# JoeMWatson/input-inference-for-control

Hardware: AMD Instinct MI355X
Metric: i2c timestep-messages/sec (cell-iterations/s = B*T*EM-iters/s), pendulum T=200 B=4096 per GPU (higher is better)
Workload: dtype f64; 1 GPU; pendulum_known_quad cubature i2c (nx=2, nu=1, nz=4), T=200, B=4096 trajectories per GPU, global batch 4096, CubatureQuadrature(1,0,0), alpha0=100, tol=0; batch_per_gpu=4096, horizon=200, parallelism=batch-sharded x1, no collective in the EM loop, kernels=one lane per trajectory

## Files before the change

### input-inference-for-control_amd/csrc/i2c_cell.hpp

```cpp
#pragma once
#include <stdint.h>
#include <type_traits>
#include "../../include/i2c_hip.h"
#include "i2c_linalg.hpp"
#include "i2c_models.hpp"
#include "i2c_random.hpp"

namespace i2c {

template <typename R> struct Rule {
  R sf;
  R w0;
  R wi;
  R W;
  int unit;
  int gh_degree, gh_points;
  R gh_x[I2C_MAX_GH_DEGREE], gh_w[I2C_MAX_GH_DEGREE];
};

template <class M> struct PerTraj : M {};
template <class M> struct is_per_traj : std::false_type {};
template <class M> struct is_per_traj<PerTraj<M>> : std::true_type {};
template <typename R, bool PER_TRAJ> struct ParamsB {};
template <typename R> struct ParamsB<R, true> {
// ... 142 lines not shown
  I2C_HD static constexpr int dep(int k) { return M::obs_dep(k); }
};
template <class M> struct TermStruct {
  I2C_HD static constexpr int lin(int k) { return M::term_lin(k); }
  I2C_HD static constexpr int dep(int k) { return M::term_dep(k); }
};
template <class M> struct MeasStruct {
  I2C_HD static constexpr int lin(int k) { return M::meas_lin(k); }
  I2C_HD static constexpr int dep(int k) { return M::meas_dep(k); }
};
template <int DIN> struct DenseStruct {
  I2C_HD static constexpr int lin(int) { return -1; }
  I2C_HD static constexpr int dep(int) { return DIN - 1; }
};

template <class M, class ST, int DIN, int DOUT, bool CROSS, bool UNITW = false, bool HANDOFF = false, typename R, class F>
I2C_FN void sp_transform(const Rule<R>& rule, const R* m, const R* Sin, const R* L, const F& f, R* my, R* Sy,
                         R* Sxy, const PolyTab<R>* tab = nullptr) {
  static_assert(!HANDOFF || (CROSS && ST::lin(0) < 0 && ST::dep(0) == DIN - 1 && ST::lin(DOUT - 1) < 0 && ST::dep(DOUT - 1) == DIN - 1),
                "the hand-off of the differences is the dense callback's");
  constexpr int NA = M::NA, NA1 = NA > 0 ? NA : 1;
  R s0[NA1], c0[NA1];
#pragma unroll
  for (int a = 0; a < NA; ++a) {
    if (tab)
      r_sincos(m[M::ang(a)], *tab, &s0[a], &c0[a]);
    else
      r_sincos(m[M::ang(a)], &s0[a], &c0[a]);
  }
  R y0[DOUT];
  f(m, s0, c0, y0);
  constexpr bool NOISE = carries_noise<F>::value;
  static_assert(!NOISE || (!HANDOFF && ST::lin(0) < 0 && ST::dep(0) == DIN - 1), "a noise term rides on a dense callback, whose every column is evaluated");
  R q0[NOISE ? sym(DOUT) : 1], qs[NOISE ? sym(DOUT) : 1];
  if constexpr (NOISE) {
    f.noise(m, s0, c0, q0);
#pragma unroll
    for (int i = 0; i < sym(DOUT); ++i) qs[i] = R(0);
  }
  R A[DOUT];
#pragma unroll
  for (int k = 0; k < DOUT; ++k) A[k] = R(0);
#pragma unroll
// ... 17 lines not shown
          xm[i] = m[i];
        } else {
          const R d = rule.sf * L[tri(i, j)];
          xp[i] = m[i] + d;
          xm[i] = m[i] - d;
        }
      }
      R sp[NA1], cp[NA1], sm[NA1], cm[NA1];
#pragma unroll
      for (int q = 0; q < NA; ++q) {
        if (M::ang(q) < j) {
          sp[q] = sm[q] = s0[q];
          cp[q] = cm[q] = c0[q];
        } else {
          R sd, cd;
          if (tab)
            r_sincos(rule.sf * L[tri(M::ang(q), j)], *tab, &sd, &cd);
          else
            r_sincos_small(rule.sf * L[tri(M::ang(q), j)], &sd, &cd);
          sp[q] = s0[q] * cd + c0[q] * sd;
          cp[q] = c0[q] * cd - s0[q] * sd;
          sm[q] = s0[q] * cd - c0[q] * sd;
          cm[q] = c0[q] * cd + s0[q] * sd;
        }
      }
      R yp[DOUT], ym[DOUT];
      f(xp, sp, cp, yp);
      f(xm, sm, cm, ym);
      if constexpr (NOISE) {
        R qp[sym(DOUT)], qm[sym(DOUT)];
        f.noise(xp, sp, cp, qp);
        f.noise(xm, sm, cm, qm);
#pragma unroll
        for (int i = 0; i < sym(DOUT); ++i) qs[i] += qp[i] + qm[i];
      }
#pragma unroll
      for (int k = 0; k < DOUT; ++k) {
        a[k] = (yp[k] - y0[k]) + (ym[k] - y0[k]);
// ... 70 lines not shown
    R v = mu[i];
#pragma unroll
    for (int k = 0; k < DZ; ++k) v += Sxz[i * DZ + k] * q[k];
    mu[i] = v;
    sched_fence<(DZ >= 8)>();
  }
#pragma unroll
  for (int i = 0; i < DX; ++i)
#pragma unroll
    for (int j = 0; j <= i; ++j) {
      R v = S[tri(i, j)];
#pragma unroll
      for (int k = 0; k < DZ; ++k) v -= Sxz[i * DZ + k] * Sxz[j * DZ + k];
      S[tri(i, j)] = v;
    }
  return ok;
}

template <int N, typename R> I2C_FN R pdf_ratio(R* S, const R* delta, bool* ok, const PolyTab<R>* tab = nullptr) {
  R rinv[N], q[N];
  *ok = chol<N>(S, rinv);
#pragma unroll
  for (int i = 0; i < N; ++i) q[i] = delta[i];
  fsub<N>(S, rinv, q);
  R maha = R(0);
#pragma unroll
  for (int i = 0; i < N; ++i) maha += q[i] * q[i];
  (void)tab;
  return r_exp(R(-0.5) * maha);
}
// ... 248 lines not shown
  return (int)__builtin_amdgcn_mbcnt_hi(~0u, __builtin_amdgcn_mbcnt_lo(~0u, 0u));
#endif
}
template <int GRID> I2C_FN bool grid_writer() {
  if constexpr (GRID == GRID_WAVE) return grid_lane() == 0;
  else return true;
}
template <int GRID> I2C_FN void grid_read_before_write() {
#ifdef I2C_HOST_SIM
  if constexpr (GRID == GRID_WAVE) grid_sim_sync();
#endif
}
template <class M, int DIN, int DOUT, bool CROSS, typename R, class F>
I2C_FN void grid_transform_wave(const Rule<R>& rule, const R* m, const R* L, const F& f, R* my, R* Sy, R* Sxy);

template <int GRID, class M, class ST, int DIN, int DOUT, bool CROSS, bool UNITW = false, bool HANDOFF = false, typename R, class F>
I2C_FN void transform(const Rule<R>& rule, const R* m, const R* Sin, const R* L, const F& f, R* my, R* Sy, R* Sxy,
                      const PolyTab<R>* tab = nullptr) {
  static_assert(!HANDOFF || GRID == 0, "the hand-off of the differences is the sigma-point rule's (sp_transform)");
  if constexpr (GRID == GRID_WAVE) {
    grid_transform_wave<M, DIN, DOUT, CROSS>(rule, m, L, f, my, Sy, Sxy);
  } else if constexpr (GRID != 0) {
    if constexpr (DIN <= 3) {
      if (rule.gh_degree == 3) return grid_transform_ct<M, 3, DIN, DOUT, CROSS>(rule, m, L, f, my, Sy, Sxy);
      if (rule.gh_degree == 4) return grid_transform_ct<M, 4, DIN, DOUT, CROSS>(rule, m, L, f, my, Sy, Sxy);
      if (rule.gh_degree == 2) return grid_transform_ct<M, 2, DIN, DOUT, CROSS>(rule, m, L, f, my, Sy, Sxy);
    }
    grid_transform<M, DIN, DOUT, CROSS>(rule, m, L, f, my, Sy, Sxy);
  } else
    sp_transform<M, ST, DIN, DOUT, CROSS, UNITW, HANDOFF>(rule, m, Sin, L, f, my, Sy, Sxy, tab);
}


template <typename R, typename S = R> struct FwdArgs {
  const S* prior;
  S* fwd;
  S* prior_out;
  const R* x0;
  const R* sig_x0;
  const R* z;
  const R* alpha;
  const R* alpha_cell;
  const uint8_t* ff;
  int32_t* status;
  const uint8_t* expert;
};

struct NoRelease {
  static constexpr bool ON = false, GAIN = false;
  int chunk_len;
  I2C_HD inline void release() const {}
  I2C_HD inline void release_if(int, int) const {}
};
struct ChunkRelease {
  static constexpr bool ON = true, GAIN = false;
  int chunk_len;
  I2C_HD inline void release() const {
#if defined(__HIP_DEVICE_COMPILE__)
    __builtin_amdgcn_fence(__ATOMIC_RELEASE, "workgroup");
    __builtin_amdgcn_s_waitcnt(0x0F70);
    __builtin_amdgcn_s_barrier();
#endif
  }
  I2C_HD inline void release_if(const int t, const int at) const {
#if defined(__HIP_DEVICE_COMPILE__)
    asm volatile("s_cmp_lg_u32 %0, %1\n\ts_cbranch_scc1 .Lnot_released_%=\n\ts_waitcnt vmcnt(0)\n\ts_barrier\n.Lnot_released_%=:"
                 :
                 : "s"(t), "s"(at)
                 : "memory", "scc");
#else
    (void)t, (void)at;
#endif
  }
};
template <typename R> struct ChunkReleaseGain {
  static constexpr bool ON = true, GAIN = true;
  int chunk_len;
  R* term_sig;
  I2C_HD inline void release() const { ChunkRelease{chunk_len}.release(); }
  I2C_HD inline void release_if(const int t, const int at) const { ChunkRelease{chunk_len}.release_if(t, at); }
};

I2C_HD inline int clamp_horizon(const int h, const int T) { return h < 1 ? 1 : (h > T ? T : h); }
template <class M, typename R, bool LEAN = false, int GRID = 0, typename ST_ = R, class REL = NoRelease, bool HZ = false>
I2C_HD inline void forward_sweep_body(const Consts<M, R>& c, const FwdArgs<R, ST_>& a, const int b, const REL rel = REL{0},
                                      [[maybe_unused]] const int Tb = 0) {
  using C = Consts<M, R>;
  constexpr int NX = C::NX, NU = C::NU, NZ = C::NZ, NZT = C::NZT, D = C::D;
  constexpr unsigned W = sizeof(ST_);
  static_assert(!HZ || (!LEAN && GRID == 0 && !REL::ON), "per-trajectory horizons: the generic one-lane sweep on its own");
  const unsigned long B = c.B;
  const int T = HZ ? Tb : c.T;
  const unsigned bo = (unsigned)b * W;
// ... 49 lines not shown
  for (int i = 0; i < sym(NX); ++i) sig_x[i] = opaque(sig_x[i]);
  const R alpha_settled = opaque(alpha_traj);
  R alpha_cur = opaque((!LEAN && a.alpha_cell) ? a.alpha_cell[(long)c.row(0) * B + b] : alpha_settled);
  constexpr bool CONST_V = VOFF && (sym(NZ) + sym(NX) <= 16);
  PolyTab<R> ptab;
  if (CONST_V) poly_tab_init(ptab);
  const PolyTab<R>* const tab = CONST_V ? &ptab : nullptr;
  R xi0_v[CONST_V ? sym(NZ) : 1], eta_v[CONST_V ? sym(NX) : 1];
  if (CONST_V) {
#pragma unroll
    for (int i = 0; i < sym(NZ); ++i) xi0_v[i] = opaque(c.sig_xi0[i]);
#pragma unroll
    for (int i = 0; i < sym(NX); ++i) eta_v[i] = opaque(LEAN ? c.sig_eta[i] : c.sig_eta_w[i]);
  }

  [[maybe_unused]] int next_release = rel.chunk_len;
  for (int t = 0; t < T; ++t) {
    const int tn = HZ ? t + 1 : (t + 1 < T ? t + 1 : t);
    [[maybe_unused]] const bool more = !HZ || t + 1 < T;
    const int tr = (LEAN || HZ) ? t : c.row(t), tnr = (LEAN || HZ) ? tn : c.row(tn);
    const unsigned rb = opaque_uniform(rb0);
    const int kz = (C::D >= 6) ? (int)opaque_uniform(0u) : 0;
    if (!PREFETCH) {
      const Window w = make_window(a.prior + (unsigned long)tr * C::E_POST * B, (unsigned long)C::E_POST * rb);
#pragma unroll
      for (int e = 0; e < C::E_PRI; ++e) pri[e] = (R)wld<ST_>(w, VOFF ? 0u : (e) * rb, VOFF ? voff[e] : bo);
#pragma unroll
      for (int k = 0; k < NZ; ++k) zt[k] = (!LEAN && c.z_per_cell) ? a.z[((long)tr * NZ + k) * B + b] : c.zg[k];
    }

// ... 96 lines not shown
#pragma unroll
      for (int e = 0; e < C::E_PRI; ++e) pri[e] = (R)wld<ST_>(w, VOFF ? 0u : (e) * rb, VOFF ? voff[e] : bo);
    }
    }

    sched_fence<(D >= 6)>();
    {
      R Lf[STRUCT_L0 ? 1 : sym(D)], rinv[D];
      if (!STRUCT_L0) {
#pragma unroll
        for (int i = 0; i < sym(D); ++i) Lf[i] = S0[i];
        cell_bad = flag_stage(cell_bad, chol<D>(Lf, rinv), 1);
      }
      const R* L = STRUCT_L0 ? L0 : Lf;
      R mz[NZ], Sz[sym(NZ)], Sxz[D * NZ];
      transform<GRID, M, ObsStruct<M>, D, NZ, true, LEAN>(c.rule_xu, mu0, S0, L, ObserveF<M, R>{params_of(c, b)}, mz, Sz, Sxz, tab);
#pragma unroll
      for (int i = 0; i < sym(NZ); ++i) Sz[i] += alpha * (CONST_V ? xi0_v[i] : c.sig_xi0[i + kz]);
      cell_bad = flag_stage(cell_bad, kalman_update<D, NZ>(mu0, S0, mz, Sz, Sxz, zt), 2);
    }
    if (!LEAN && PREFETCH && c.z_per_cell && more) {
#pragma unroll
      for (int k = 0; k < NZ; ++k) zt[k] = a.z[((long)tnr * NZ + k) * B + b];
    }
    const Window out = make_window(a.fwd + (unsigned long)t * C::E_FWD * B, (unsigned long)C::E_FWD * rb);
    if (wr) {
#pragma unroll
      for (int e = 0; e < D; ++e) wst(out, VOFF ? 0u : (e) * rb, VOFF ? voff[e] : bo, (ST_)mu0[e]);
#pragma unroll
      for (int e = 0; e < sym(D); ++e) wst(out, VOFF ? 0u : (D + e) * rb, VOFF ? voff[D + e] : bo, (ST_)S0[e]);
    }

    sched_fence<(D >= 6)>();
    R Sxy[D * NX];
    constexpr bool NOISE = GRID == 0 && has_process_noise<M, R>::value;
    static_assert(!NOISE || !REL::ON, "a model with process_noise runs the plain sweep (Impl::launches)");
    [[maybe_unused]] R qn[NOISE ? sym(NX) : 1];
    {
      R L[sym(D)], rinv[D];
#pragma unroll
      for (int i = 0; i < sym(D); ++i) L[i] = S0[i];
      cell_bad = flag_stage(cell_bad, chol<D>(L, rinv), 3);
      if constexpr (NOISE)
        transform<GRID, M, DenseStruct<D>, D, NX, true, LEAN>(c.rule_xu, mu0, S0, L, DynamicsNoiseF<M, R>{{params_of(c, b)}, qn}, mu_x, sig_x, Sxy, tab);
      else
        transform<GRID, M, DenseStruct<D>, D, NX, true, LEAN, REL::GAIN>(c.rule_xu, mu0, S0, L, DynamicsF<M, R>{params_of(c, b)}, mu_x, sig_x, Sxy, tab);
    }
#pragma unroll
    for (int i = 0; i < sym(NX); ++i) sig_x[i] += CONST_V ? eta_v[i] : (LEAN ? c.sig_eta[i + kz] : c.sig_eta_w[i + kz]);
    if constexpr (NOISE) {
#pragma unroll
      for (int i = 0; i < sym(NX); ++i) sig_x[i] += qn[i];
    }
    R L3[sym(NX)], rinv3[NX];
#pragma unroll
    for (int i = 0; i < sym(NX); ++i) L3[i] = sig_x[i];
    cell_bad = flag_stage(cell_bad, chol<NX>(L3, rinv3), 4);
    sched_fence<(D >= 6)>();
    if constexpr (!REL::GAIN) {
#pragma unroll
// ... 36 lines not shown
        }
      }
      transform<GRID, M, TermStruct<M>, NX, NT, true, LEAN>(c.rule_x, mu_x, sig_x, L3, ObserveTermF<M, R>{params_of(c, b)}, mzt, Szt, Sxzt);
#pragma unroll
      for (int i = 0; i < sym(NT); ++i) Szt[i] += alpha * c.sig_xiT0[i];
      cell_bad = flag_stage(cell_bad, kalman_update<NX, NT>(mu_x, sig_x, mzt, Szt, Sxzt, c.zg_term), 5);
      if (STRUCT_L0) {
#pragma unroll
        for (int i = 0; i < sym(NX); ++i) L3[i] = sig_x[i];
        cell_bad = flag_stage(cell_bad, chol<NX>(L3, rinv3), 5);
      }
    }
    if (STRUCT_L0) {
#pragma unroll
      for (int i = 0; i < sym(NX); ++i) Lx[i] = L3[i];
    }
    fail = fold_cell_failure(fail, cell_bad, t);
    if (wr) {
#pragma unroll
      for (int e = 0; e < NX; ++e)
        wst(out, VOFF ? 0u : (D + sym(D) + e) * rb, VOFF ? voff[D + sym(D) + e] : bo, (ST_)(e == 0 ? nan_if(fail != 0, mu_x[e]) : mu_x[e]));
#pragma unroll
      for (int e = 0; e < sym(NX); ++e) wst(out, VOFF ? 0u : (D + sym(D) + NX + e) * rb, VOFF ? voff[D + sym(D) + NX + e] : bo, (ST_)sig_x[e]);
    }

  }
  if constexpr (REL::ON) rel.release();
  if (wr && fail != 0 && a.status[b] == 0) a.status[b] = fail;
}

// ... 1690 lines not shown
```

### input-inference-for-control_amd/csrc/i2c_impl.hpp

```cpp
#pragma once
#include "i2c_entry.hpp"
#include "i2c_cell.hpp"
#include "i2c_group.hpp"
#include "i2c_wave.hpp"
#include "i2c_quad.hpp"
#include "i2c_grid.hpp"
#include "i2c_linearize.hpp"

#include <cmath>
#include <cstdio>
#include <cstdlib>
#include <cstring>

namespace i2c {

constexpr int SWEEP_BLOCK = 64;
#ifndef I2C_LANE_BLOCK
#define I2C_LANE_BLOCK 64
#endif
constexpr int LANE_BLOCK = I2C_LANE_BLOCK;
constexpr int CELL_BLOCK = 256;

#ifdef I2C_HOST_SIM
#define I2C_KERNEL(BLOCK) static void
// ... 283 lines not shown
  pm.term_stats[B + b] = m;
  pm.term_stats[2 * B + b] = v;
  Consts<M, R> cm = c;
  cm.tol = pm.tol;
  mstep_update<M, R>(cm, pm.ms, b, trT, m, v, m, alpha);
}
template <class M, typename R, bool LEAN, typename S = R>
I2C_KERNEL(LANE_BLOCK) k_forward_mstep(I2C_LANE_PARAMS const Consts<M, R> c, const FwdArgs<R, S> a, const int block, const PendingMstep<R> pm) {
  const long b = I2C_LANE_X(block);
  if (b < c.B) {
    finish_pending_mstep<M, R>(c, pm, (int)b);
    forward_sweep_body<M, R, LEAN, 0, S>(c, a, (int)b);
  }
}

template <class M, typename R, bool LEAN, typename S, bool MSTEP, bool GAINH>
I2C_FN void forward_helper_lane(const Consts<M, R>& c, const FwdArgs<R, S>& a, const ChunkArgs<R, S>& ch, const PendingMstep<R>& pm,
                                const int role, const int b) {
  if constexpr (GAINH) {
    static_assert(sizeof(S) == sizeof(R), "the gain hand-off is not rounded to a narrower storage type");
    R* const term_sig = ch.part;
    if (role == 0) {
      if constexpr (MSTEP) finish_pending_mstep<M, R>(c, pm, b);
      forward_sweep_body<M, R, LEAN, 0, S, ChunkReleaseGain<R>>(c, a, b, ChunkReleaseGain<R>{ch.chunk_len, term_sig});
    } else {
      for (int k = 0; k < ch.n_chunks; ++k) {
#if defined(__HIP_DEVICE_COMPILE__)
        __builtin_amdgcn_s_barrier();
        __builtin_amdgcn_fence(__ATOMIC_ACQUIRE, "workgroup");
#endif
        chunk_compose_gain_body<M, R>(c, ch, term_sig, k, b);
      }
    }
  } else if (role == 0) {
    if constexpr (MSTEP) finish_pending_mstep<M, R>(c, pm, b);
    forward_sweep_body<M, R, LEAN, 0, S, ChunkRelease>(c, a, b, ChunkRelease{ch.chunk_len});
  } else {
    for (int k = 0; k < ch.n_chunks; ++k) {
#if defined(__HIP_DEVICE_COMPILE__)
      __builtin_amdgcn_s_barrier();
      __builtin_amdgcn_fence(__ATOMIC_ACQUIRE, "workgroup");
#endif
      chunk_compose_body<M, R, S>(c, ch, k, b);
    }
  }
}
#ifdef I2C_HOST_SIM
constexpr int HELPER_WAVES = 1;
#define I2C_HELPER_LANES                                                                \
  const long b = I2C_LANE_X(LANE_BLOCK);                                                \
  for (int role = 0; role < 2; ++role)
#else
constexpr int HELPER_WAVES = 2;
#define I2C_HELPER_LANES                                                                \
  const long b = (long)blockIdx.x * LANE_BLOCK + (threadIdx.x & (LANE_BLOCK - 1));      \
  const int role = __builtin_amdgcn_readfirstlane((int)(threadIdx.x / LANE_BLOCK));     \
  if (b < c.B)
#endif
template <class M, typename R, bool LEAN, typename S = R, bool GAINH = false>
I2C_KERNEL(2 * LANE_BLOCK) k_forward_helper(I2C_LANE_PARAMS const Consts<M, R> c, const FwdArgs<R, S> a, const ChunkArgs<R, S> ch) {
  I2C_HELPER_LANES forward_helper_lane<M, R, LEAN, S, false, GAINH>(c, a, ch, PendingMstep<R>{}, role, (int)b);
}
template <class M, typename R, bool LEAN, typename S = R, bool GAINH = false>
I2C_KERNEL(2 * LANE_BLOCK) k_forward_mstep_helper(I2C_LANE_PARAMS const Consts<M, R> c, const FwdArgs<R, S> a, const ChunkArgs<R, S> ch,
                                                  const PendingMstep<R> pm) {
  I2C_HELPER_LANES forward_helper_lane<M, R, LEAN, S, true, GAINH>(c, a, ch, pm, role, (int)b);
}
#undef I2C_HELPER_LANES


template <typename R> static bool unit_rule(const Rule<R>& r) { return r.unit && r.w0 == R(0); }
template <class M, typename R> static bool unit_rule(const Consts<M, R>& c) { return unit_rule(c.rule_xu) && unit_rule(c.rule_x); }

#ifdef I2C_HOST_SIM
template <typename R, class Body>
static void sim_teams(const int team, const long n_teams, const int n_rows, const bool rows_on_team, const size_t lds, const Body& body) {
  for (int y0 = 0; y0 < (rows_on_team ? 1 : n_rows); ++y0)
    for (long i = 0; i < n_teams; ++i) {
      std::vector<R> sh(lds, R(0)), xch(128, R(0));
      HostBarrier bar(team);
      std::vector<std::thread> lanes;
      for (int l = 0; l < team; ++l)
// ... 498 lines not shown
template <class M, typename R, typename S> static ChunkArgs<R, S> chunk_args(const I2cProblem* p, const CellArgs<R, S>& a) {
  ChunkArgs<R, S> ch{a, (R*)p->work, nullptr, nullptr, 0, 0};
  chunk_geometry(p->B, p->T, &ch.n_chunks, &ch.chunk_len);
  const ChunkWork<M> w(p->B, ch.n_chunks);
  ch.bnd = ch.comp + w.bnd;
  ch.part = ch.comp + w.part;
  return ch;
}

#define I2C_MODEL_CONST(name, MEMBER, DEFAULT)                                                                      \
  template <class M, class = void> struct name : std::integral_constant<int, (DEFAULT)> {};                         \
  template <class M> struct name<M, std::void_t<decltype(M::MEMBER)>> : std::integral_constant<int, M::MEMBER> {};
I2C_MODEL_CONST(bwd_fused_min_b, BWD_FUSED_MIN_B, I2C_BWD_FUSED_MIN_B)
I2C_MODEL_CONST(forward_helper_min_b, FORWARD_HELPER_MIN_B, 4096)
I2C_MODEL_CONST(forward_helper_gain, FORWARD_HELPER_GAIN, M::NX + M::NU <= 3)
I2C_MODEL_CONST(quad_backward_min_b, QUAD_BACKWARD8_MIN_B, 0)
I2C_MODEL_CONST(quad_backward_max_b, QUAD_BACKWARD8_MAX_B, -1)
I2C_MODEL_CONST(quad_chunk_walk_min_b, QUAD_CHUNK_WALK_MIN_B, 0)
I2C_MODEL_CONST(quad_chunk_walk_max_b, QUAD_CHUNK_WALK_MAX_B, -1)
I2C_MODEL_CONST(quad_chunk_passes_min_b, QUAD_CHUNK_PASSES_MIN_B, 0)
I2C_MODEL_CONST(quad_chunk_passes_max_b, QUAD_CHUNK_PASSES_MAX_B, -1)
I2C_MODEL_CONST(quad_chunk_stitch_max_b, QUAD_CHUNK_STITCH_MAX_B, -1)
#undef I2C_MODEL_CONST


struct Plan {
  int forward, backward, propagate, filter;
  int schedule;
  int walker;
  int compose, stitch;
  int rule;
  bool fwd_tm;
  bool fusable;
};
struct Launches {
  const int schedule;
  const bool self_stitch;
  const bool helper;
  const bool helper_gain;
  const bool defer;
  const bool reduces;
  const bool walk_lean;
};

template <class M, typename R, typename S = R> struct Impl {
  using C = Consts<M, R>;
  static constexpr bool MIXED = sizeof(S) != sizeof(R);
  static constexpr int G = M::GROUP;
  static constexpr bool NOISE = has_process_noise<M, R>::value;
  static constexpr bool HAS_GROUP = G > 0 && sizeof(R) == 8 && !MIXED && !NOISE;
  static constexpr bool LANE = !M::GROUP_ONLY;
  static constexpr bool HAS_WAVE = M::WAVE && sizeof(R) == 8 && !NOISE;
  static constexpr bool HAS_QUAD = M::QUAD && sizeof(R) == 8 && !(NOISE && QG<M>::WIDE);
  static constexpr bool WIDE = QG<M>::WIDE;
  static constexpr bool HAS_QUAD_BACKWARD = HAS_QUAD && quad_backward_exists<M>();
  static constexpr bool QUAD8 = HAS_QUAD_BACKWARD && !WIDE && LANE;
  static constexpr bool HAS_QUAD_CKF = HAS_QUAD && !MIXED && quad_ckf_exists<M>();
// ... 259 lines not shown
    return q;
  }
  static C forward_consts(const I2cProblem* p) { return make_consts<M, R>(p, 0.0, p->inference == I2C_INF_LINEARIZE ? p->expert_controller : 0); }
  static C propagate_consts(const I2cProblem* p, const int use_expert) {
    if (p->inference != I2C_INF_LINEARIZE) return make_consts<M, R>(p, 0.0, use_expert);
    const I2cProblem q = with_unit_rule(p);
    return make_consts<M, R>(&q, 0.0, use_expert);
  }
  static C filter_consts(const I2cProblem* p) {
    I2cProblem q = with_unit_rule(p);
    q.inference = I2C_INF_CUBATURE;
    return make_consts<M, R>(&q, 0.0, 0);
  }

  static constexpr bool SELF_STITCH = LANE && C::D <= 5;
  static Launches launches(const I2cProblem* p, const Plan& pl, const C& c, const void* xm, const void* zpost, const void* cell_stats,
                           const bool in_learn) {
    const int mode = schedule_with(pl, p->work != nullptr);
    const bool chunked = mode == I2C_BWD_CHUNKED;
    const bool two_launch = SELF_STITCH && chunked && pl.rule == I2C_INF_CUBATURE && !c.has_x_terminal && !chunk_four_passes();
    const bool self = two_launch && pl.stitch == I2C_FAMILY_LANE && pl.walker == I2C_FAMILY_LANE;
    const bool lane_forward = in_learn && two_launch && pl.forward == I2C_FAMILY_LANE;
    bool helper = !NOISE && lane_forward && pl.compose == I2C_FAMILY_LANE && LANE_BLOCK == 64 && sweep_lanes() == LANE_BLOCK;
    if (helper) {
      const char* e = getenv("I2C_FORWARD_HELPER");
      helper = e ? strcmp(e, "0") != 0 : p->B >= forward_helper_min_b<M>::value;
    }
    const bool reduces = pl.backward == I2C_FAMILY_WAVE   ? mode == I2C_BWD_TWO_PASS && xm && cell_stats
                         : pl.backward == I2C_FAMILY_LANE ? mode != I2C_BWD_FUSED
                                                          : chunked;
    const char* const eg = getenv("I2C_FORWARD_HELPER_GAIN");
    int n_chunks, chunk_len;
    chunk_geometry(p->B, p->T, &n_chunks, &chunk_len);
    const bool helper_gain = helper && !MIXED && 3 * n_chunks >= sym(C::NX) && (eg ? strcmp(eg, "0") != 0 : forward_helper_gain<M>::value != 0);
    return Launches{mode, self, helper, helper_gain, !NOISE && lane_forward && self, reduces, I2C_WALK_LEAN && !xm && !zpost && !cell_stats && !c.z_per_cell};
  }

  template <bool LEAN>
  static int launch_forward_lane(const I2cProblem* p, const Launches& L, const C& c, const FwdArgs<R, S>& a, const PendingMstep<R>& pend, void* stream) {
    const int lanes = sweep_lanes();
    if constexpr (SELF_STITCH && !NOISE) {
      if (L.helper) {
        constexpr int W = HELPER_WAVES;
        const ChunkArgs<R, S> ch = chunk_args<M>(p, CellArgs<R, S>{a.fwd});
        if constexpr (!MIXED) {
          if (L.helper_gain)
            return pend.part ? launch(k_forward_mstep_helper<M, R, LEAN, S, true>, W * (long)p->B, 1, W * LANE_BLOCK, stream, c, a, ch, pend)
                             : launch(k_forward_helper<M, R, LEAN, S, true>, W * (long)p->B, 1, W * LANE_BLOCK, stream, c, a, ch);
        }
        return pend.part ? launch(k_forward_mstep_helper<M, R, LEAN, S>, W * (long)p->B, 1, W * LANE_BLOCK, stream, c, a, ch, pend)
                         : launch(k_forward_helper<M, R, LEAN, S>, W * (long)p->B, 1, W * LANE_BLOCK, stream, c, a, ch);
      }
      if (pend.part) return launch(k_forward_mstep<M, R, LEAN, S>, p->B, 1, lanes, stream, c, a, lanes, pend);
    }
    return launch(k_forward<M, R, LEAN, false, S>, p->B, 1, lanes, stream, c, a, lanes);
  }
  static int run_forward(const I2cProblem* p, const Plan& pl, const Launches& L, const C& c, const void* prior, void* fwd, void* prior_out,
                         int32_t* status, void* stream, const PendingMstep<R>& pend = {}) {
    if (pl.forward < 0) return pl.forward;
// ... 14 lines not shown
      }
    }
    if (pl.forward == I2C_FAMILY_GROUP) {
      if constexpr (HAS_GROUP) return launch_group<GK_FORWARD, M, R, G>(c, nullptr, a, stream);
    }
    if (pl.forward == I2C_FAMILY_GRID) {
      if constexpr (HAS_GRID) return launch_grid<GRK_FORWARD, M, R>(c, a, stream);
    }
    if constexpr (LANE) {
      if constexpr (!MIXED) {
        if (pl.rule == I2C_INF_LINEARIZE) return launch(k_forward_lin<M, R>, p->B, 1, LANE_BLOCK, stream, c, a);
        if (pl.rule == I2C_INF_GAUSS_HERMITE) return launch(k_forward<M, R, false, true>, p->B, 1, LANE_BLOCK, stream, c, a, LANE_BLOCK);
      }
      const bool lean = c.rule_xu.unit && c.rule_x.unit && !c.z_per_cell && !a.alpha_cell && !a.prior_out && c.t0 == 0;
      if (plan_trace())
        fprintf(stderr, "i2c_forward_lane: sweep=%s lean=%d gain=%s\n", L.helper ? "helper" : "plain", (int)lean, L.helper_gain ? "helper" : "sweep");
      return lean ? launch_forward_lane<true>(p, L, c, a, pend, stream) : launch_forward_lane<false>(p, L, c, a, pend, stream);
    }
    return I2C_ENOTSUP;
  }
  static int forward(const I2cProblem* p, const void* prior, void* fwd, void* prior_out, int32_t* status, void* stream) {
    const Plan pl = resolve(p);
    const C c = forward_consts(p);
    return run_forward(p, pl, launches(p, pl, c, nullptr, nullptr, nullptr, false), c, prior, fwd, prior_out, status, stream);
  }

  static const R* terminal_alpha(const I2cProblem* p, const C& c) {
    return p->alpha_cell ? (const R*)p->alpha_cell + (long)c.row(p->T - 1) * (long)p->B : (const R*)p->alpha;
  }
  static MstepArgs<R> mstep_args(const I2cProblem* p, const void* term_stats, void* stats_out, const int update = 1) {
    return MstepArgs<R>{(const R*)term_stats, (R*)p->alpha, (R*)stats_out, update};
// ... 395 lines not shown
```

Measured before the change: 2.494 billion timestep-messages/s.

## Offload forward-sweep sincos to dedicated trig server waves via LDS mailbox

Adds two extra server waves per block that compute the sin/cos of the pendulum angle and its sigma-point offsets. The sweep wave posts the mean and offsets to an LDS mailbox early, right after the leading rows of the Kalman update, and collects the results later through inline-asm polling with a timeout. The intent is to take the fp64 transcendental latency off the serial per-trajectory critical path and overlap it with the remaining update work. In exchange the block grows to four waves, uses more LDS and adds spin-wait synchronisation, which can cost occupancy or stall the sweep if the servers fall behind.

```diff
diff --git a/input-inference-for-control_amd/csrc/i2c_cell.hpp b/input-inference-for-control_amd/csrc/i2c_cell.hpp
--- a/input-inference-for-control_amd/csrc/i2c_cell.hpp
+++ b/input-inference-for-control_amd/csrc/i2c_cell.hpp
@@ -180,19 +180,128 @@
   I2C_HD static constexpr int dep(int) { return DIN - 1; }
 };
 
-template <class M, class ST, int DIN, int DOUT, bool CROSS, bool UNITW = false, bool HANDOFF = false, typename R, class F>
+constexpr int TRIG_NARG = 2;
+constexpr unsigned TRIG_ROW = 64 * 8, TRIG_SLOT = 3 * TRIG_NARG * TRIG_ROW, TRIG_RES = TRIG_NARG * TRIG_ROW, TRIG_WORDS = 4 * TRIG_SLOT,
+                   TRIG_BOX_BYTES = TRIG_WORDS + 32, TRIG_POLL_TICKS = 10000000u, TRIG_DEAD = 0x40000000u;
+constexpr unsigned trig_slot(int e, int srv) { return (unsigned)(2 * e + srv) * TRIG_SLOT; }
+constexpr unsigned trig_arg_word(int e, int srv) { return TRIG_WORDS + 4u * (unsigned)(2 * e + srv); }
+constexpr unsigned trig_res_word(int e, int srv) { return TRIG_WORDS + 16u + 4u * (unsigned)(2 * e + srv); }
+template <class ST, int DOUT> constexpr int trig_cols() {
+  int cols = 0;
+  for (int k = 0; k < DOUT; ++k)
+    if (ST::lin(k) < 0 && ST::dep(k) + 1 > cols) cols = ST::dep(k) + 1;
+  return cols;
+}
+template <class M, class ST, int DOUT> constexpr int trig_noff() {
+  const int cols = trig_cols<ST, DOUT>();
+  return cols == 0 ? 0 : (M::ang(0) < cols ? M::ang(0) + 1 : cols);
+}
+struct TrigState {
+  unsigned lane, box, seq, limit;
+};
+struct TrigHere {
+  static constexpr bool MAIL = false;
+  static constexpr int NOFF = 1;
+};
+template <int E, int NOFF_> struct TrigMail {
+  static constexpr bool MAIL = true;
+  static constexpr int NOFF = NOFF_;
+  static_assert(NOFF >= 1 && NOFF <= TRIG_NARG, "one or two offsets per transform");
+  TrigState* st;
+  template <typename R> I2C_HD inline void post(const R mean, const R* off) const {
+#if defined(__HIP_DEVICE_COMPILE__)
+    static_assert(sizeof(R) == 8, "the trig waves serve the fp64 sweep");
+    const unsigned seq_v = st->seq;
+    if constexpr (NOFF == 1)
+      asm volatile("ds_write_b64 %0, %2 offset:%5\n\tds_write_b64 %0, %3 offset:%6\n\ts_waitcnt lgkmcnt(0)\n\t"
+                   "ds_write_b32 %1, %4 offset:%7\n\tds_write_b32 %1, %4 offset:%8"
+                   :
+                   : "v"(st->lane), "v"(st->box), "v"(mean), "v"(off[0]), "v"(seq_v), "n"(trig_slot(E, 0)), "n"(trig_slot(E, 1)),
+                     "n"(trig_arg_word(E, 0)), "n"(trig_arg_word(E, 1))
+                   : "memory");
+    else
+      asm volatile("ds_write_b64 %0, %2 offset:%6\n\tds_write_b64 %0, %3 offset:%7\n\tds_write_b64 %0, %4 offset:%8\n\t"
+                   "s_waitcnt lgkmcnt(0)\n\tds_write_b32 %1, %5 offset:%9\n\tds_write_b32 %1, %5 offset:%10"
+                   :
+                   : "v"(st->lane), "v"(st->box), "v"(mean), "v"(off[0]), "v"(off[1]), "v"(seq_v), "n"(trig_slot(E, 0)),
+                     "n"(trig_slot(E, 1)), "n"(trig_slot(E, 1) + TRIG_ROW), "n"(trig_arg_word(E, 0)), "n"(trig_arg_word(E, 1))
+                   : "memory");
+#else
+    (void)mean, (void)off;
+#endif
+  }
+  template <typename R> I2C_HD inline void collect(R* s0, R* c0, R* sd, R* cd) const {
+#if defined(__HIP_DEVICE_COMPILE__)
+    static_assert(sizeof(R) == 8, "the trig waves serve the fp64 sweep");
+    unsigned w0, w1, u0, u1, t0;
+    unsigned seq = uniform_u32(st->seq), limit = uniform_u32(st->limit);
+#define I2C_TRIG_LOOK(READS)                                                                                              \
+  "ds_read_b32 %[w0], %[box] offset:%[rw0]\n\tds_read_b32 %[w1], %[box] offset:%[rw1]\n\t" READS
+#define I2C_TRIG_MATCH                                                                                                    \
+  "s_waitcnt lgkmcnt(0)\n\tv_readfirstlane_b32 %[u0], %[w0]\n\tv_readfirstlane_b32 %[u1], %[w1]\n\t"                      \
+  "s_min_u32 %[u0], %[u0], %[u1]\n\ts_cmp_eq_u32 %[u0], %[seq]\n\ts_cbranch_scc1 .Ltrig_have_%=\n\t"
+#define I2C_TRIG_COLLECT(READS, NANS)                                                                                     \
+  I2C_TRIG_LOOK(READS) I2C_TRIG_MATCH                                                                                     \
+  "s_memtime vcc\n\ts_waitcnt lgkmcnt(0)\n\ts_mov_b32 %[t0], vcc_lo\n"                                                    \
+  ".Ltrig_poll_%=:\n\t" I2C_TRIG_LOOK(READS) "s_memtime vcc\n\t" I2C_TRIG_MATCH                                           \
+  "s_sub_u32 %[u0], vcc_lo, %[t0]\n\ts_cmp_lt_u32 %[u0], %[lim]\n\ts_cbranch_scc1 .Ltrig_poll_%=\n\t"                     \
+  "s_or_b32 %[seq], %[seq], %[dead]\n\ts_mov_b32 %[lim], 0\n\t" NANS "\n.Ltrig_have_%=:"
+    if constexpr (NOFF == 1) {
+      asm volatile(I2C_TRIG_COLLECT("ds_read_b64 %[a], %[lane] offset:%[r0]\n\tds_read_b64 %[b], %[lane] offset:%[r0b]\n\t"
+                                    "ds_read_b64 %[c], %[lane] offset:%[r1]\n\tds_read_b64 %[d], %[lane] offset:%[r1b]\n\t",
+                                    "v_mov_b64 %[a], -1\n\tv_mov_b64 %[b], -1\n\tv_mov_b64 %[c], -1\n\tv_mov_b64 %[d], -1")
+                   : [a] "=&v"(s0[0]), [b] "=&v"(c0[0]), [c] "=&v"(sd[0]), [d] "=&v"(cd[0]), [w0] "=&v"(w0), [w1] "=&v"(w1),
+                     [u0] "=&s"(u0), [u1] "=&s"(u1), [t0] "=&s"(t0), [seq] "+s"(seq), [lim] "+s"(limit)
+                   : [lane] "v"(st->lane), [box] "v"(st->box), [dead] "n"(TRIG_DEAD),
+                     [r0] "n"(trig_slot(E, 0) + TRIG_RES), [r0b] "n"(trig_slot(E, 0) + TRIG_RES + TRIG_ROW),
+                     [r1] "n"(trig_slot(E, 1) + TRIG_RES), [r1b] "n"(trig_slot(E, 1) + TRIG_RES + TRIG_ROW),
+                     [r1c] "n"(trig_slot(E, 1) + TRIG_RES + 2 * TRIG_ROW), [r1d] "n"(trig_slot(E, 1) + TRIG_RES + 3 * TRIG_ROW), [rw0] "n"(trig_res_word(E, 0)),
+                     [rw1] "n"(trig_res_word(E, 1))
+                   : "memory", "scc", "vcc");
+    } else {
+      asm volatile(I2C_TRIG_COLLECT("ds_read_b64 %[a], %[lane] offset:%[r0]\n\tds_read_b64 %[b], %[lane] offset:%[r0b]\n\t"
+                                    "ds_read_b64 %[c], %[lane] offset:%[r1]\n\tds_read_b64 %[d], %[lane] offset:%[r1b]\n\t"
+                                    "ds_read_b64 %[e], %[lane] offset:%[r1c]\n\tds_read_b64 %[f], %[lane] offset:%[r1d]\n\t",
+                                    "v_mov_b64 %[a], -1\n\tv_mov_b64 %[b], -1\n\tv_mov_b64 %[c], -1\n\tv_mov_b64 %[d], -1\n\t"
+                                    "v_mov_b64 %[e], -1\n\tv_mov_b64 %[f], -1")
+                   : [a] "=&v"(s0[0]), [b] "=&v"(c0[0]), [c] "=&v"(sd[0]), [d] "=&v"(cd[0]), [e] "=&v"(sd[1]), [f] "=&v"(cd[1]),
+                     [w0] "=&v"(w0), [w1] "=&v"(w1), [u0] "=&s"(u0), [u1] "=&s"(u1), [t0] "=&s"(t0), [seq] "+s"(seq), [lim] "+s"(limit)
+                   : [lane] "v"(st->lane), [box] "v"(st->box), [dead] "n"(TRIG_DEAD),
+                     [r0] "n"(trig_slot(E, 0) + TRIG_RES), [r0b] "n"(trig_slot(E, 0) + TRIG_RES + TRIG_ROW),
+                     [r1] "n"(trig_slot(E, 1) + TRIG_RES), [r1b] "n"(trig_slot(E, 1) + TRIG_RES + TRIG_ROW),
+                     [r1c] "n"(trig_slot(E, 1) + TRIG_RES + 2 * TRIG_ROW), [r1d] "n"(trig_slot(E, 1) + TRIG_RES + 3 * TRIG_ROW), [rw0] "n"(trig_res_word(E, 0)),
+                     [rw1] "n"(trig_res_word(E, 1))
+                   : "memory", "scc", "vcc");
+    }
+    st->seq = seq, st->limit = limit;
+#undef I2C_TRIG_COLLECT
+#undef I2C_TRIG_MATCH
+#undef I2C_TRIG_LOOK
+#else
+    (void)s0, (void)c0, (void)sd, (void)cd;
+#endif
+  }
+};
+
+template <class M, class ST, int DIN, int DOUT, bool CROSS, bool UNITW = false, bool HANDOFF = false, typename R, class F, class TS = TrigHere>
 I2C_FN void sp_transform(const Rule<R>& rule, const R* m, const R* Sin, const R* L, const F& f, R* my, R* Sy,
-                         R* Sxy, const PolyTab<R>* tab = nullptr) {
+                         R* Sxy, const PolyTab<R>* tab = nullptr, [[maybe_unused]] const TS* ts = nullptr) {
   static_assert(!HANDOFF || (CROSS && ST::lin(0) < 0 && ST::dep(0) == DIN - 1 && ST::lin(DOUT - 1) < 0 && ST::dep(DOUT - 1) == DIN - 1),
                 "the hand-off of the differences is the dense callback's");
   constexpr int NA = M::NA, NA1 = NA > 0 ? NA : 1;
   R s0[NA1], c0[NA1];
-#pragma unroll
-  for (int a = 0; a < NA; ++a) {
-    if (tab)
-      r_sincos(m[M::ang(a)], *tab, &s0[a], &c0[a]);
-    else
-      r_sincos(m[M::ang(a)], &s0[a], &c0[a]);
+  [[maybe_unused]] R sd_mail[TS::NOFF], cd_mail[TS::NOFF];
+  if constexpr (TS::MAIL) {
+    static_assert(NA == 1 && TS::NOFF == trig_noff<M, ST, DOUT>(), "one model angle, and the offsets of the columns that move it");
+    ts->collect(s0, c0, sd_mail, cd_mail);
+  } else {
+#pragma unroll
+    for (int a = 0; a < NA; ++a) {
+      if (tab)
+        r_sincos(m[M::ang(a)], *tab, &s0[a], &c0[a]);
+      else
+        r_sincos(m[M::ang(a)], &s0[a], &c0[a]);
+    }
   }
   R y0[DOUT];
   f(m, s0, c0, y0);
@@ -240,14 +349,27 @@
           cp[q] = cm[q] = c0[q];
         } else {
           R sd, cd;
-          if (tab)
-            r_sincos(rule.sf * L[tri(M::ang(q), j)], *tab, &sd, &cd);
-          else
-            r_sincos_small(rule.sf * L[tri(M::ang(q), j)], &sd, &cd);
-          sp[q] = s0[q] * cd + c0[q] * sd;
-          cp[q] = c0[q] * cd - s0[q] * sd;
-          sm[q] = s0[q] * cd - c0[q] * sd;
-          cm[q] = c0[q] * cd + s0[q] * sd;
+          if constexpr (TS::MAIL) {
+            sd = sd_mail[j < TS::NOFF ? j : 0];
+            cd = cd_mail[j < TS::NOFF ? j : 0];
+          } else {
+            if (tab)
+              r_sincos(rule.sf * L[tri(M::ang(q), j)], *tab, &sd, &cd);
+            else
+              r_sincos_small(rule.sf * L[tri(M::ang(q), j)], &sd, &cd);
+          }
+          if constexpr (TS::MAIL) {
+            const R s0cd = s0[q] * cd, s0sd = s0[q] * sd;
+            sp[q] = m_fma(c0[q], sd, s0cd);
+            cp[q] = m_fma(c0[q], cd, -s0sd);
+            sm[q] = m_fma(-c0[q], sd, s0cd);
+            cm[q] = m_fma(c0[q], cd, s0sd);
+          } else {
+            sp[q] = s0[q] * cd + c0[q] * sd;
+            cp[q] = c0[q] * cd - s0[q] * sd;
+            sm[q] = s0[q] * cd - c0[q] * sd;
+            cm[q] = c0[q] * cd + s0[q] * sd;
+          }
         }
       }
       R yp[DOUT], ym[DOUT];
@@ -348,6 +470,41 @@
       for (int k = 0; k < DZ; ++k) v -= Sxz[i * DZ + k] * Sxz[j * DZ + k];
       S[tri(i, j)] = v;
     }
+  return ok;
+}
+
+template <int DX, int DZ, int LEAD, typename R, class HOOK>
+I2C_FN bool kalman_update_lead(R* mu, R* S, const R* mz, R* Sz, R* Sxz, const R* zt, const HOOK& hook) {
+  static_assert(LEAD >= 1 && LEAD <= DX, "the leading rows are rows of the state");
+  R rinv[DZ];
+  const bool ok = chol<DZ>(Sz, rinv);
+  R q[DZ];
+#pragma unroll
+  for (int k = 0; k < DZ; ++k) q[k] = zt[k] - mz[k];
+  fsub<DZ>(Sz, rinv, q);
+#pragma unroll
+  for (int part = 0; part < 2; ++part) {
+    const int lo = part ? LEAD : 0, hi = part ? DX : LEAD;
+#pragma unroll
+    for (int i = lo; i < hi; ++i) {
+      fsub<DZ>(Sz, rinv, &Sxz[i * DZ]);
+      R v = mu[i];
+#pragma unroll
+      for (int k = 0; k < DZ; ++k) v += Sxz[i * DZ + k] * q[k];
+      mu[i] = v;
+      sched_fence<(DZ >= 8)>();
+    }
+#pragma unroll
+    for (int i = lo; i < hi; ++i)
+#pragma unroll
+      for (int j = 0; j <= i; ++j) {
+        R v = S[tri(i, j)];
+#pragma unroll
+        for (int k = 0; k < DZ; ++k) v -= Sxz[i * DZ + k] * Sxz[j * DZ + k];
+        S[tri(i, j)] = v;
+      }
+    if (part == 0) hook(mu, S);
+  }
   return ok;
 }
 
@@ -626,9 +783,10 @@
 template <class M, int DIN, int DOUT, bool CROSS, typename R, class F>
 I2C_FN void grid_transform_wave(const Rule<R>& rule, const R* m, const R* L, const F& f, R* my, R* Sy, R* Sxy);
 
-template <int GRID, class M, class ST, int DIN, int DOUT, bool CROSS, bool UNITW = false, bool HANDOFF = false, typename R, class F>
+template <int GRID, class M, class ST, int DIN, int DOUT, bool CROSS, bool UNITW = false, bool HANDOFF = false, typename R, class F, class TS = TrigHere>
 I2C_FN void transform(const Rule<R>& rule, const R* m, const R* Sin, const R* L, const F& f, R* my, R* Sy, R* Sxy,
-                      const PolyTab<R>* tab = nullptr) {
+                      const PolyTab<R>* tab = nullptr, const TS* ts = nullptr) {
+  static_assert(!TS::MAIL || GRID == 0, "the trig waves serve the sigma-point rule (sp_transform)");
   static_assert(!HANDOFF || GRID == 0, "the hand-off of the differences is the sigma-point rule's (sp_transform)");
   if constexpr (GRID == GRID_WAVE) {
     grid_transform_wave<M, DIN, DOUT, CROSS>(rule, m, L, f, my, Sy, Sxy);
@@ -640,7 +798,7 @@
     }
     grid_transform<M, DIN, DOUT, CROSS>(rule, m, L, f, my, Sy, Sxy);
   } else
-    sp_transform<M, ST, DIN, DOUT, CROSS, UNITW, HANDOFF>(rule, m, Sin, L, f, my, Sy, Sxy, tab);
+    sp_transform<M, ST, DIN, DOUT, CROSS, UNITW, HANDOFF>(rule, m, Sin, L, f, my, Sy, Sxy, tab, ts);
 }
 
 
@@ -659,13 +817,13 @@
 };
 
 struct NoRelease {
-  static constexpr bool ON = false, GAIN = false;
+  static constexpr bool ON = false, GAIN = false, TRIG = false;
   int chunk_len;
   I2C_HD inline void release() const {}
   I2C_HD inline void release_if(int, int) const {}
 };
 struct ChunkRelease {
-  static constexpr bool ON = true, GAIN = false;
+  static constexpr bool ON = true, GAIN = false, TRIG = false;
   int chunk_len;
   I2C_HD inline void release() const {
 #if defined(__HIP_DEVICE_COMPILE__)
@@ -686,9 +844,17 @@
   }
 };
 template <typename R> struct ChunkReleaseGain {
-  static constexpr bool ON = true, GAIN = true;
+  static constexpr bool ON = true, GAIN = true, TRIG = false;
   int chunk_len;
   R* term_sig;
+  I2C_HD inline void release() const { ChunkRelease{chunk_len}.release(); }
+  I2C_HD inline void release_if(const int t, const int at) const { ChunkRelease{chunk_len}.release_if(t, at); }
+};
+template <typename R> struct ChunkReleaseGainTrig {
+  static constexpr bool ON = true, GAIN = true, TRIG = true;
+  int chunk_len;
+  R* term_sig;
+  unsigned trig_lane, trig_box;
   I2C_HD inline void release() const { ChunkRelease{chunk_len}.release(); }
   I2C_HD inline void release_if(const int t, const int at) const { ChunkRelease{chunk_len}.release_if(t, at); }
 };
@@ -768,6 +934,20 @@
     for (int i = 0; i < sym(NX); ++i) eta_v[i] = opaque(LEAN ? c.sig_eta[i] : c.sig_eta_w[i]);
   }
 
+  constexpr int TRIG_OBS = REL::TRIG ? trig_noff<M, ObsStruct<M>, NZ>() : 0, TRIG_DYN = REL::TRIG ? trig_noff<M, DenseStruct<D>, NX>() : 0;
+  using TrigObs = TrigMail<0, TRIG_OBS ? TRIG_OBS : 1>;
+  using TrigDyn = TrigMail<1, TRIG_DYN ? TRIG_DYN : 1>;
+  [[maybe_unused]] TrigState trig{0, 0, TRIG_OBS ? 1u : 2u, TRIG_POLL_TICKS};
+  if constexpr (REL::TRIG) {
+    static_assert(GRID == 0 && STRUCT_L0 && !HZ && M::NA == 1 && M::ang(0) < NX && TRIG_DYN >= 1, "the trig waves' window (Impl::launches)");
+    trig.lane = rel.trig_lane, trig.box = rel.trig_box;
+    if constexpr (TRIG_OBS > 0) {
+      R off[TRIG_OBS];
+#pragma unroll
+      for (int j = 0; j < TRIG_OBS; ++j) off[j] = c.rule_xu.sf * Lx[tri(M::ang(0), j)];
+      TrigObs{&trig}.post(mu_x[M::ang(0)], off);
+    }
+  }
   [[maybe_unused]] int next_release = rel.chunk_len;
   for (int t = 0; t < T; ++t) {
     const int tn = HZ ? t + 1 : (t + 1 < T ? t + 1 : t);
@@ -894,10 +1074,28 @@
       }
       const R* L = STRUCT_L0 ? L0 : Lf;
       R mz[NZ], Sz[sym(NZ)], Sxz[D * NZ];
-      transform<GRID, M, ObsStruct<M>, D, NZ, true, LEAN>(c.rule_xu, mu0, S0, L, ObserveF<M, R>{params_of(c, b)}, mz, Sz, Sxz, tab);
+      if constexpr (TRIG_OBS > 0) {
+        const TrigObs mail{&trig};
+        transform<GRID, M, ObsStruct<M>, D, NZ, true, LEAN>(c.rule_xu, mu0, S0, L, ObserveF<M, R>{params_of(c, b)}, mz, Sz, Sxz, tab, &mail);
+        trig.seq += 1;
+      } else
+        transform<GRID, M, ObsStruct<M>, D, NZ, true, LEAN>(c.rule_xu, mu0, S0, L, ObserveF<M, R>{params_of(c, b)}, mz, Sz, Sxz, tab);
 #pragma unroll
       for (int i = 0; i < sym(NZ); ++i) Sz[i] += alpha * (CONST_V ? xi0_v[i] : c.sig_xi0[i + kz]);
-      cell_bad = flag_stage(cell_bad, kalman_update<D, NZ>(mu0, S0, mz, Sz, Sxz, zt), 2);
+      if constexpr (REL::TRIG) {
+        const auto post_dyn = [&](const R* mu1, const R* S1) {
+          constexpr int A1 = M::ang(0) + 1;
+          R Lh[sym(A1)], rh[A1], off[TRIG_DYN];
+#pragma unroll
+          for (int i = 0; i < sym(A1); ++i) Lh[i] = S1[i];
+          (void)chol<A1>(Lh, rh);
+#pragma unroll
+          for (int j = 0; j < TRIG_DYN; ++j) off[j] = c.rule_xu.sf * Lh[tri(M::ang(0), j)];
+          TrigDyn{&trig}.post(mu1[M::ang(0)], off);
+        };
+        cell_bad = flag_stage(cell_bad, kalman_update_lead<D, NZ, M::ang(0) + 1>(mu0, S0, mz, Sz, Sxz, zt, post_dyn), 2);
+      } else
+        cell_bad = flag_stage(cell_bad, kalman_update<D, NZ>(mu0, S0, mz, Sz, Sxz, zt), 2);
     }
     if (!LEAN && PREFETCH && c.z_per_cell && more) {
 #pragma unroll
@@ -924,6 +1122,11 @@
       if constexpr (NOISE)
         transform<GRID, M, DenseStruct<D>, D, NX, true, LEAN>(c.rule_xu, mu0, S0, L, DynamicsNoiseF<M, R>{{params_of(c, b)}, qn}, mu_x, sig_x, Sxy, tab);
       else
+        if constexpr (REL::TRIG) {
+        const TrigDyn mail{&trig};
+        transform<GRID, M, DenseStruct<D>, D, NX, true, LEAN, REL::GAIN>(c.rule_xu, mu0, S0, L, DynamicsF<M, R>{params_of(c, b)}, mu_x, sig_x, Sxy, tab, &mail);
+        trig.seq += TRIG_OBS ? 1 : 2;
+      } else
         transform<GRID, M, DenseStruct<D>, D, NX, true, LEAN, REL::GAIN>(c.rule_xu, mu0, S0, L, DynamicsF<M, R>{params_of(c, b)}, mu_x, sig_x, Sxy, tab);
     }
 #pragma unroll
@@ -990,6 +1193,12 @@
     if (STRUCT_L0) {
 #pragma unroll
       for (int i = 0; i < sym(NX); ++i) Lx[i] = L3[i];
+    }
+    if constexpr (TRIG_OBS > 0) {
+      R off[TRIG_OBS];
+#pragma unroll
+      for (int j = 0; j < TRIG_OBS; ++j) off[j] = c.rule_xu.sf * Lx[tri(M::ang(0), j)];
+      TrigObs{&trig}.post(mu_x[M::ang(0)], off);
     }
     fail = fold_cell_failure(fail, cell_bad, t);
     if (wr) {
diff --git a/input-inference-for-control_amd/csrc/i2c_impl.hpp b/input-inference-for-control_amd/csrc/i2c_impl.hpp
--- a/input-inference-for-control_amd/csrc/i2c_impl.hpp
+++ b/input-inference-for-control_amd/csrc/i2c_impl.hpp
@@ -321,10 +321,99 @@
   }
 }
 
-template <class M, typename R, bool LEAN, typename S, bool MSTEP, bool GAINH>
+template <class M, typename R, int SRV, int NOBS, int NDYN>
+I2C_FN void trig_server_lane([[maybe_unused]] const int T, [[maybe_unused]] const int chunk_len, [[maybe_unused]] double* const box) {
+#if defined(__HIP_DEVICE_COMPILE__)
+  static_assert(sizeof(R) == 8 && NOBS <= TRIG_NARG && NDYN <= TRIG_NARG, "the trig waves serve the fp64 sweep");
+  PolyTab<R> tab;
+  poly_tab_init(tab);
+  typedef __attribute__((address_space(3))) double lds_f64;
+  typedef __attribute__((address_space(3))) unsigned lds_u32;
+  const unsigned lane = threadIdx.x & (LANE_BLOCK - 1);
+  lds_f64* const lbox = (lds_f64*)box;
+  lds_u32* const words = (lds_u32*)(lbox + TRIG_WORDS / 8);
+  bool dead = false;
+  int next_release = chunk_len;
+  for (int t = 0; t < T; ++t) {
+#pragma unroll
+    for (int e = 0; e < 2; ++e) {
+      const int n = SRV == 0 ? ((e ? NDYN : NOBS) > 0 ? 1 : 0) : (e ? NDYN : NOBS);
+      if (n > 0 && !dead) {
+        const unsigned seq = 2u * (unsigned)t + (unsigned)e + 1u;
+        lds_u32* const aw = words + (2 * e + SRV);
+        volatile lds_f64* const slot = lbox + trig_slot(e, SRV) / 8 + lane;
+        const unsigned t0 = (unsigned)__builtin_amdgcn_s_memtime();
+        while ((unsigned)__builtin_amdgcn_readfirstlane((int)__hip_atomic_load(aw, __ATOMIC_ACQUIRE, __HIP_MEMORY_SCOPE_WORKGROUP)) != seq) {
+          if ((unsigned)__builtin_amdgcn_s_memtime() - t0 >= TRIG_POLL_TICKS) {
+            dead = true;
+            break;
+          }
+        }
+        if (!dead) {
+          R sn[TRIG_NARG], cs[TRIG_NARG];
+#pragma unroll
+          for (int k = 0; k < n; ++k) r_sincos((R)slot[k * 64], tab, &sn[k], &cs[k]);
+#pragma unroll
+          for (int k = 0; k < n; ++k) {
+            slot[(TRIG_NARG + 2 * k) * 64] = sn[k];
+            slot[(TRIG_NARG + 2 * k + 1) * 64] = cs[k];
+          }
+          __hip_atomic_store(words + 4 + (2 * e + SRV), seq, __ATOMIC_RELEASE, __HIP_MEMORY_SCOPE_WORKGROUP);
+        }
+      }
+    }
+    if (t == next_release) {
+      __builtin_amdgcn_s_barrier();
+      next_release += chunk_len;
+    }
+  }
+  __builtin_amdgcn_s_barrier();
+#endif
+}
+template <class M, typename R, bool LEAN, typename S, bool MSTEP, bool GAINH, bool TRIG = false>
 I2C_FN void forward_helper_lane(const Consts<M, R>& c, const FwdArgs<R, S>& a, const ChunkArgs<R, S>& ch, const PendingMstep<R>& pm,
-                                const int role, const int b) {
-  if constexpr (GAINH) {
+                                const int role, const int b, [[maybe_unused]] double* const box = nullptr) {
+  if constexpr (TRIG) {
+    static_assert(GAINH && sizeof(S) == sizeof(R), "the trig waves ride on the gain hand-off");
+    using C = Consts<M, R>;
+    constexpr int NOBS = trig_noff<M, ObsStruct<M>, C::NZ>(), NDYN = trig_noff<M, DenseStruct<C::D>, C::NX>();
+    R* const term_sig = ch.part;
+    [[maybe_unused]] unsigned lane_addr = 0, box_addr = 0;
+#if defined(__HIP_DEVICE_COMPILE__)
+    typedef __attribute__((address_space(3))) unsigned char lds_byte;
+    box_addr = (unsigned)(unsigned long)(lds_byte*)box;
+    lane_addr = box_addr + 8u * (threadIdx.x & (LANE_BLOCK - 1));
+    if (role == 0) {
+      __builtin_amdgcn_s_setprio(3);
+      unsigned* const words = reinterpret_cast<unsigned*>(box + TRIG_WORDS / 8);
+#pragma unroll
+      for (int i = 0; i < 8; ++i) words[i] = 0u;
+      __builtin_amdgcn_fence(__ATOMIC_RELEASE, "workgroup");
+    }
+    __builtin_amdgcn_s_barrier();
+    __builtin_amdgcn_fence(__ATOMIC_ACQUIRE, "workgroup");
+#endif
+    if (role == 0) {
+      if constexpr (MSTEP) finish_pending_mstep<M, R>(c, pm, b);
+#ifdef I2C_HOST_SIM
+      forward_sweep_body<M, R, LEAN, 0, S, ChunkReleaseGain<R>>(c, a, b, ChunkReleaseGain<R>{ch.chunk_len, term_sig});
+#else
+      forward_sweep_body<M, R, LEAN, 0, S, ChunkReleaseGainTrig<R>>(c, a, b, ChunkReleaseGainTrig<R>{ch.chunk_len, term_sig, lane_addr, box_addr});
+#endif
+    } else if (role == 1) {
+      for (int k = 0; k < ch.n_chunks; ++k) {
+#if defined(__HIP_DEVICE_COMPILE__)
+        __builtin_amdgcn_s_barrier();
+        __builtin_amdgcn_fence(__ATOMIC_ACQUIRE, "workgroup");
+#endif
+        chunk_compose_gain_body<M, R>(c, ch, term_sig, k, b);
+      }
+    } else if (role == 2) {
+      trig_server_lane<M, R, 0, NOBS, NDYN>(c.T, ch.chunk_len, box);
+    } else {
+      trig_server_lane<M, R, 1, NOBS, NDYN>(c.T, ch.chunk_len, box);
+    }
+  } else if constexpr (GAINH) {
     static_assert(sizeof(S) == sizeof(R), "the gain hand-off is not rounded to a narrower storage type");
     R* const term_sig = ch.part;
     if (role == 0) {
@@ -353,12 +442,14 @@
   }
 }
 #ifdef I2C_HOST_SIM
-constexpr int HELPER_WAVES = 1;
+constexpr int HELPER_WAVES = 1, TRIG_WAVES = 1;
+#define I2C_TRIG_BOX double* const box = nullptr;
 #define I2C_HELPER_LANES                                                                \
   const long b = I2C_LANE_X(LANE_BLOCK);                                                \
   for (int role = 0; role < 2; ++role)
 #else
-constexpr int HELPER_WAVES = 2;
+constexpr int HELPER_WAVES = 2, TRIG_WAVES = 4;
+#define I2C_TRIG_BOX __shared__ double box[TRIG_BOX_BYTES / 8];
 #define I2C_HELPER_LANES                                                                \
   const long b = (long)blockIdx.x * LANE_BLOCK + (threadIdx.x & (LANE_BLOCK - 1));      \
   const int role = __builtin_amdgcn_readfirstlane((int)(threadIdx.x / LANE_BLOCK));     \
@@ -373,6 +464,18 @@
                                                   const PendingMstep<R> pm) {
   I2C_HELPER_LANES forward_helper_lane<M, R, LEAN, S, true, GAINH>(c, a, ch, pm, role, (int)b);
 }
+template <class M, typename R, bool LEAN>
+I2C_KERNEL(4 * LANE_BLOCK) k_forward_trig(I2C_LANE_PARAMS const Consts<M, R> c, const FwdArgs<R, R> a, const ChunkArgs<R, R> ch) {
+  I2C_TRIG_BOX
+  I2C_HELPER_LANES forward_helper_lane<M, R, LEAN, R, false, true, true>(c, a, ch, PendingMstep<R>{}, role, (int)b, box);
+}
+template <class M, typename R, bool LEAN>
+I2C_KERNEL(4 * LANE_BLOCK) k_forward_mstep_trig(I2C_LANE_PARAMS const Consts<M, R> c, const FwdArgs<R, R> a, const ChunkArgs<R, R> ch,
+                                                const PendingMstep<R> pm) {
+  I2C_TRIG_BOX
+  I2C_HELPER_LANES forward_helper_lane<M, R, LEAN, R, true, true, true>(c, a, ch, pm, role, (int)b, box);
+}
+#undef I2C_TRIG_BOX
 #undef I2C_HELPER_LANES
 
 
@@ -901,6 +1004,7 @@
 I2C_MODEL_CONST(bwd_fused_min_b, BWD_FUSED_MIN_B, I2C_BWD_FUSED_MIN_B)
 I2C_MODEL_CONST(forward_helper_min_b, FORWARD_HELPER_MIN_B, 4096)
 I2C_MODEL_CONST(forward_helper_gain, FORWARD_HELPER_GAIN, M::NX + M::NU <= 3)
+I2C_MODEL_CONST(forward_helper_trig, FORWARD_HELPER_TRIG, M::NX + M::NU <= 3)
 I2C_MODEL_CONST(quad_backward_min_b, QUAD_BACKWARD8_MIN_B, 0)
 I2C_MODEL_CONST(quad_backward_max_b, QUAD_BACKWARD8_MAX_B, -1)
 I2C_MODEL_CONST(quad_chunk_walk_min_b, QUAD_CHUNK_WALK_MIN_B, 0)
@@ -928,6 +1032,7 @@
   const bool defer;
   const bool reduces;
   const bool walk_lean;
+  const bool helper_trig;
 };
 
 template <class M, typename R, typename S = R> struct Impl {
@@ -1217,6 +1322,11 @@
   }
 
   static constexpr bool SELF_STITCH = LANE && C::D <= 5;
+  static constexpr bool trig_window() {
+    if constexpr (M::NA == 1) return M::ang(0) < C::NX && M::ang(0) < TRIG_NARG;
+    return false;
+  }
+  static constexpr bool TRIG_WINDOW = SELF_STITCH && !NOISE && !MIXED && sizeof(R) == 8 && trig_window();
   static Launches launches(const I2cProblem* p, const Plan& pl, const C& c, const void* xm, const void* zpost, const void* cell_stats,
                            const bool in_learn) {
     const int mode = schedule_with(pl, p->work != nullptr);
@@ -1236,7 +1346,13 @@
     int n_chunks, chunk_len;
     chunk_geometry(p->B, p->T, &n_chunks, &chunk_len);
     const bool helper_gain = helper && !MIXED && 3 * n_chunks >= sym(C::NX) && (eg ? strcmp(eg, "0") != 0 : forward_helper_gain<M>::value != 0);
-    return Launches{mode, self, helper, helper_gain, !NOISE && lane_forward && self, reduces, I2C_WALK_LEAN && !xm && !zpost && !cell_stats && !c.z_per_cell};
+    bool helper_trig = false;
+    if constexpr (TRIG_WINDOW) {
+      const char* const et = getenv("I2C_FORWARD_HELPER_TRIG");
+      helper_trig = helper_gain && !p->horizons && (et ? strcmp(et, "0") != 0 : forward_helper_trig<M>::value != 0);
+    }
+    return Launches{mode, self, helper, helper_gain, !NOISE && lane_forward && self, reduces, I2C_WALK_LEAN && !xm && !zpost && !cell_stats && !c.z_per_cell,
+                    helper_trig};
   }
 
   template <bool LEAN>
@@ -1246,6 +1362,11 @@
       if (L.helper) {
         constexpr int W = HELPER_WAVES;
         const ChunkArgs<R, S> ch = chunk_args<M>(p, CellArgs<R, S>{a.fwd});
+        if constexpr (TRIG_WINDOW) {
+          if (L.helper_trig)
+            return pend.part ? launch(k_forward_mstep_trig<M, R, LEAN>, TRIG_WAVES * (long)p->B, 1, TRIG_WAVES * LANE_BLOCK, stream, c, a, ch, pend)
+                             : launch(k_forward_trig<M, R, LEAN>, TRIG_WAVES * (long)p->B, 1, TRIG_WAVES * LANE_BLOCK, stream, c, a, ch);
+        }
         if constexpr (!MIXED) {
           if (L.helper_gain)
             return pend.part ? launch(k_forward_mstep_helper<M, R, LEAN, S, true>, W * (long)p->B, 1, W * LANE_BLOCK, stream, c, a, ch, pend)
@@ -1290,7 +1411,8 @@
       }
       const bool lean = c.rule_xu.unit && c.rule_x.unit && !c.z_per_cell && !a.alpha_cell && !a.prior_out && c.t0 == 0;
       if (plan_trace())
-        fprintf(stderr, "i2c_forward_lane: sweep=%s lean=%d gain=%s\n", L.helper ? "helper" : "plain", (int)lean, L.helper_gain ? "helper" : "sweep");
+        fprintf(stderr, "i2c_forward_lane: sweep=%s lean=%d gain=%s trig=%s\n", L.helper ? "helper" : "plain", (int)lean,
+                L.helper_gain ? "helper" : "sweep", L.helper_trig ? "waves" : "sweep");
       return lean ? launch_forward_lane<true>(p, L, c, a, pend, stream) : launch_forward_lane<false>(p, L, c, a, pend, stream);
     }
     return I2C_ENOTSUP;
```

Result: no change. 2.507 billion timestep-messages/s, median of 6 (+0.5%).
